# Twilight-Dream-Of-Magic/KolmogorovLike-DataCompressor

Hardware: AMD Instinct MI355X
Metric: compress MB/s at fixed block size, bit-exact vs reference; 1/2/4/8-GPU scaling (higher is better)
Workload: dtype u8; 1 GPU; enwik-style synthetic text (kolm.datagen.enwik_like, seed 20251212+rank), 256 MiB per GPU resident in HBM, 1 MiB fixed blocks, candidates 0..8 + MDL, payloads emitted in HBM; block_size=1048576, bytes_per_gpu=268435456, blocks_per_gpu=256, parallelism=block-shard x1

## Files before the change

### kolmogorovlike-datacompressor_amd/csrc/k_mtf.hip

```cpp
#include "kolm_internal.h"

namespace kolm {

namespace {

struct ChunkGeom {
    Geom geo;
    u32 cpb;
    u32 csz;
    __device__ inline bool range(u32 c, u32& lo, u32& hi) const {
        const u32 b = c / cpb;
        const u32 k = c - b * cpb;
        lo = geo.base(b) + k * csz;
        const u32 e = geo.end(b);
        hi = min(lo + csz, e);
        return lo < e;
    }
};

constexpr u32 MTF_SLAB = 64;

__global__ __launch_bounds__(256) void k_mtf_summary(ChunkGeom cg, const u8* in, u8* summary,
                                                     u16* scnt, u32 nchunks) {
    __shared__ u32 sl[256 * MTF_SLAB / 4];
    __shared__ u32 slo[256];
    const u32 t = threadIdx.x;
    const u32 c = blockIdx.x * blockDim.x + t;
    u32 lo = 0, hi = 0;
    const bool valid = c < nchunks && cg.range(c, lo, hi);
    u16 cnt = 0;
    if (__syncthreads_and(valid && hi - lo == cg.csz && (lo & 15) == 0)) {
        u32 seen[8] = {0, 0, 0, 0, 0, 0, 0, 0};
        u8* out = summary + (u64)c * 256;
        slo[t] = lo;
        __syncthreads();
        for (u32 r = cg.csz; r > 0; r -= MTF_SLAB) {
#pragma unroll
            for (u32 q = 0; q < MTF_SLAB / 16; ++q) {
                const u32 m = q * 256 + t, owner = m >> 2, part = m & 3;
                reinterpret_cast<uint4*>(sl)[m] =
                    *reinterpret_cast<const uint4*>(in + slo[owner] + r - MTF_SLAB + 16 * part);
            }
            __syncthreads();
            const u32* slab = sl + t * (MTF_SLAB / 4);
#pragma unroll
            for (int q = MTF_SLAB / 4 - 1; q >= 0; --q) {
                const u32 wv = slab[q];
#pragma unroll
                for (int j = 3; j >= 0; --j) {
                    const u32 b = (wv >> (8 * j)) & 0xFF, w = b >> 5, bit = 1u << (b & 31);
                    u32 sw = 0;
#pragma unroll
                    for (int k = 0; k < 8; ++k) sw = (k == (int)w) ? seen[k] : sw;
                    if (!(sw & bit)) {
#pragma unroll
                        for (int k = 0; k < 8; ++k)
                            if (k == (int)w) seen[k] |= bit;
                        out[cnt++] = (u8)b;
                    }
                }
            }
            __syncthreads();
        }
        scnt[c] = cnt;
        return;
    }
    if (!valid) {
        if (c < nchunks) scnt[c] = 0;
        return;
    }
    {
        u32 seen[8] = {0, 0, 0, 0, 0, 0, 0, 0};
        u8* out = summary + (u64)c * 256;
        auto visit = [&](u32 b) {
            const u32 w = b >> 5, bit = 1u << (b & 31);
            u32 sw = 0;
#pragma unroll
            for (int k = 0; k < 8; ++k) sw = (k == (int)w) ? seen[k] : sw;
            if (!(sw & bit)) {
#pragma unroll
                for (int k = 0; k < 8; ++k)
                    if (k == (int)w) seen[k] |= bit;
                out[cnt++] = (u8)b;
            }
        };
        if (((lo | hi) & 15) == 0) {
            for (u32 i = hi; i > lo; i -= 16) {
                const uint4 v = *reinterpret_cast<const uint4*>(in + i - 16);
                const u32 wv[4] = {v.x, v.y, v.z, v.w};
#pragma unroll
                for (int q = 3; q >= 0; --q)
#pragma unroll
                    for (int j = 3; j >= 0; --j) visit((wv[q] >> (8 * j)) & 0xFF);
            }
        } else {
            for (u32 i = hi; i > lo; --i) visit(in[i - 1]);
        }
    }
    scnt[c] = cnt;
}

__device__ inline void mtf_apply(u32* st, u8* nst, u32* member, const u8* sm, u32 cnt) {
    const u32 lane = threadIdx.x & 63;
    if (lane < 8) member[lane] = 0;
    __builtin_amdgcn_wave_barrier();
    __builtin_amdgcn_fence(__ATOMIC_RELEASE, "wavefront");
    u32 sv[4];
#pragma unroll
    for (int j = 0; j < 4; ++j) {
        const u32 i = 4 * lane + j;
        sv[j] = i < cnt ? sm[i] : 0;
        if (i < cnt) atomicOr(&member[sv[j] >> 5], 1u << (sv[j] & 31));
    }
    __builtin_amdgcn_fence(__ATOMIC_ACQ_REL, "wavefront");
    __builtin_amdgcn_wave_barrier();
    const u32 word = st[lane];
    u32 keep = 0;
    u8 e[4];
#pragma unroll
    for (int j = 0; j < 4; ++j) {
        e[j] = (word >> (8 * j)) & 0xFF;
        const bool in_sum = (member[e[j] >> 5] >> (e[j] & 31)) & 1u;
        keep |= (in_sum ? 0u : 1u) << j;
    }
    const u32 nk = __popc(keep);
    u32 pos = cnt + wave_incl_scan(nk, OpAddU(), 0u) - nk;
#pragma unroll
    for (int j = 0; j < 4; ++j) {
        const u32 i = 4 * lane + j;
        if (i < cnt) nst[i] = (u8)sv[j];
        if ((keep >> j) & 1u) nst[pos++] = e[j];
    }
    __builtin_amdgcn_fence(__ATOMIC_ACQ_REL, "wavefront");
    __builtin_amdgcn_wave_barrier();
    st[lane] = reinterpret_cast<const u32*>(nst)[lane];
    __builtin_amdgcn_fence(__ATOMIC_ACQ_REL, "wavefront");
    __builtin_amdgcn_wave_barrier();
}


constexpr u32 CP_W = 16;
constexpr u32 CP_G = 8;
constexpr u32 CP_S = 16;
constexpr u32 CP_R = CP_G * CP_S;

__device__ inline u32 mtf_ident(u32 lane) {
    return (4 * lane) | ((4 * lane + 1) << 8) | ((4 * lane + 2) << 16) | ((4 * lane + 3) << 24);
}

__device__ inline void cp_range(const ChunkGeom& cg, u32 b, u32 r, u32& k0, u32& k1) {
    const u32 nch = (cg.geo.end(b) - cg.geo.base(b) + cg.csz - 1) / cg.csz;
    const u32 per = (nch + CP_R - 1) / CP_R;
    k0 = min(r * per, nch);
    k1 = min(k0 + per, nch);
}

__global__ __launch_bounds__(64 * CP_W) void k_mtf_cp1(ChunkGeom cg, const u8* summary, const u16* scnt, u32* rst,
                                                      u32* rdist) {
    __shared__ u32 st[CP_W][64];
    __shared__ u8 nst[CP_W][256];
    __shared__ u32 member[CP_W][8];
    __shared__ u32 uni[CP_W][8];
    const u32 lane = threadIdx.x & 63, w = threadIdx.x >> 6;
    const u32 gr = blockIdx.x * CP_W + w, b = gr / CP_R, r = gr - b * CP_R;
    if (b >= cg.geo.nb) return;
    u32 k0, k1;
    cp_range(cg, b, r, k0, k1);
    st[w][lane] = mtf_ident(lane);
    if (lane < 8) uni[w][lane] = 0;
    __builtin_amdgcn_wave_barrier();
    for (u32 k = k0; k < k1; ++k) {
        const u32 c = b * cg.cpb + k;
        const u8* sm = summary + (u64)c * 256;
        const u32 cnt = scnt[c];
#pragma unroll
        for (int j = 0; j < 4; ++j) {
            const u32 i = 4 * lane + j;
            if (i < cnt) atomicOr(&uni[w][sm[i] >> 5], 1u << (sm[i] & 31));
        }
        mtf_apply(st[w], nst[w], member[w], sm, cnt);
    }
    __builtin_amdgcn_fence(__ATOMIC_ACQ_REL, "wavefront");
    __builtin_amdgcn_wave_barrier();
    rst[(u64)gr * 64 + lane] = st[w][lane];
    if (lane == 0) {
        u32 d = 0;
        for (int q = 0; q < 8; ++q) d += __popc(uni[w][q]);
        rdist[gr] = d;
    }
}

__global__ __launch_bounds__(64 * CP_G) void k_mtf_cp2(const u32* rst, const u32* rdist, u32* rentry) {
    __shared__ u32 st[CP_G][64];
    __shared__ u8 nst[CP_G][256];
    __shared__ u32 member[CP_G][8];
    __shared__ u32 uni[CP_G][8];
    __shared__ u8 gsum[CP_G][256];
    __shared__ u32 gentry[CP_G][64];
    __shared__ u32 gdist[CP_G];
    const u32 lane = threadIdx.x & 63, g = threadIdx.x >> 6, b = blockIdx.x;
    const u64 r0 = (u64)b * CP_R + g * CP_S;
    st[g][lane] = mtf_ident(lane);
    if (lane < 8) uni[g][lane] = 0;
    __builtin_amdgcn_wave_barrier();
    for (u32 v = 0; v < CP_S; ++v) {
        const u8* sm = reinterpret_cast<const u8*>(rst + (r0 + v) * 64);
        const u32 cnt = rdist[r0 + v];
#pragma unroll
        for (int j = 0; j < 4; ++j) {
            const u32 i = 4 * lane + j;
            if (i < cnt) atomicOr(&uni[g][sm[i] >> 5], 1u << (sm[i] & 31));
        }
        mtf_apply(st[g], nst[g], member[g], sm, cnt);
    }
    __builtin_amdgcn_fence(__ATOMIC_ACQ_REL, "wavefront");
    __builtin_amdgcn_wave_barrier();
    reinterpret_cast<u32*>(gsum[g])[lane] = st[g][lane];
    if (lane == 0) {
        u32 d = 0;
        for (int q = 0; q < 8; ++q) d += __popc(uni[g][q]);
        gdist[g] = d;
    }
    __syncthreads();
    if (g == 0) {
        st[0][lane] = mtf_ident(lane);
        __builtin_amdgcn_wave_barrier();
        for (u32 v = 0; v < CP_G; ++v) {
            gentry[v][lane] = st[0][lane];
            __builtin_amdgcn_fence(__ATOMIC_ACQ_REL, "wavefront");
            __builtin_amdgcn_wave_barrier();
            if (v + 1 < CP_G) mtf_apply(st[0], nst[0], member[0], gsum[v], gdist[v]);
        }
    }
    __syncthreads();
    st[g][lane] = gentry[g][lane];
    __builtin_amdgcn_wave_barrier();
    for (u32 v = 0; v < CP_S; ++v) {
        rentry[(r0 + v) * 64 + lane] = st[g][lane];
        mtf_apply(st[g], nst[g], member[g], reinterpret_cast<const u8*>(rst + (r0 + v) * 64), rdist[r0 + v]);
    }
}

__global__ __launch_bounds__(64 * CP_W) void k_mtf_cp3(ChunkGeom cg, const u8* summary, const u16* scnt,
                                                      const u32* rentry, u8* states) {
    __shared__ u32 st[CP_W][64];
    __shared__ u8 nst[CP_W][256];
    __shared__ u32 member[CP_W][8];
    const u32 lane = threadIdx.x & 63, w = threadIdx.x >> 6;
    const u32 gr = blockIdx.x * CP_W + w, b = gr / CP_R, r = gr - b * CP_R;
    if (b >= cg.geo.nb) return;
    u32 k0, k1;
    cp_range(cg, b, r, k0, k1);
    st[w][lane] = rentry[(u64)gr * 64 + lane];
    __builtin_amdgcn_wave_barrier();
    for (u32 k = k0; k < k1; ++k) {
        const u32 c = b * cg.cpb + k;
        reinterpret_cast<u32*>(states + (u64)c * 256)[lane] = st[w][lane];
        mtf_apply(st[w], nst[w], member[w], summary + (u64)c * 256, scnt[c]);
    }
}

constexpr int RT = 128;

struct RiceAcc {
    u32 c[5] = {0, 0, 0, 0, 0};
    int k;
    u32 kk = 0, km = 0;
    __device__ inline void init(int rk) {
        k = rk;
        kk = rk < 8 ? (u32)rk : 0u;
        km = rk < 8 ? (0xFFu >> rk) * 0x01010101u : 0u;
    }
    __device__ inline u32 rb(u32 v) const { return (v >> k) + 1 + k; }
    __device__ inline u32 sum4(u32 w, u32 a) const { return __builtin_amdgcn_sad_u8((w >> kk) & km, 0u, a); }
    __device__ inline void add(u32 v) {
        c[0] += rb(v);
        c[2] += rb(((v & 0x0Fu) << 4) | (v >> 4));
        c[3] += rb(__brev(v) >> 24);
        c[4] += rb(v ^ (v >> 1));
    }
    __device__ inline void add4(u32 o) {
        const u32 one = 4 * (1 + k);
        c[0] = sum4(o, c[0] + one);
        c[2] = sum4(((o & 0x0F0F0F0Fu) << 4) | ((o >> 4) & 0x0F0F0F0Fu), c[2] + one);
        c[3] = sum4(__brev(o), c[3] + one);
        c[4] = sum4(o ^ ((o >> 1) & 0x7F7F7F7Fu), c[4] + one);
    }
    __device__ inline void group(u32 lo, u32 hi) {
        u64 x = ((u64)__builtin_bswap32(lo) << 32) | __builtin_bswap32(hi);
        u64 t = (x ^ (x >> 7)) & 0x00AA00AA00AA00AAull;
        x ^= t ^ (t << 7);
        t = (x ^ (x >> 14)) & 0x0000CCCC0000CCCCull;
        x ^= t ^ (t << 14);
        t = (x ^ (x >> 28)) & 0x00000000F0F0F0F0ull;
        x ^= t ^ (t << 28);
        c[1] = sum4((u32)(x >> 32), sum4((u32)x, c[1] + 8 * (1 + k)));
    }
};

__global__ __launch_bounds__(RT) void k_mtf_replay(ChunkGeom cg, const u8* in, const u8* states, u8* out,
                                                   u32 nchunks, u64* bits, int rice_k) {
    __shared__ u32 tab[64 * RT];
    const u32 t = threadIdx.x;
    const u32 c = blockIdx.x * RT + t;
    u32 lo = 0, hi = 0;
    const bool valid = c < nchunks && cg.range(c, lo, hi);
    u32 r0 = 0, r1 = 0;
    if (valid) {
        const u32* s = reinterpret_cast<const u32*>(states + (u64)c * 256);
        r0 = s[0];
        r1 = s[1];
        for (int w = 2; w < 64; ++w) tab[w * RT + t] = s[w];
    }
    auto haszero = [](u32 y) { return (y - 0x01010101u) & ~y & 0x80808080u; };
    auto front = [](u32 x, u32 j, u32 in) {
        const u32 lowmask = j ? ((1u << (8 * j)) - 1) : 0u;
        const u32 highmask = j == 3 ? 0u : ~((1u << (8 * (j + 1))) - 1);
        return (x & highmask) | ((x & lowmask) << 8) | in;
    };
    auto step = [&](u32 b) -> u32 {
        const u32 bb = b * 0x01010101u;
        u32 z = haszero(r0 ^ bb);
        if (z) {
            const u32 j = (__ffs(z) - 1) >> 3;
            r0 = front(r0, j, b);
            return j;
        }
        const u32 c0 = r0 >> 24;
        z = haszero(r1 ^ bb);
        if (z) {
            const u32 j = (__ffs(z) - 1) >> 3;
            r0 = (r0 << 8) | b;
            r1 = front(r1, j, c0);
            return 4 + j;
        }
        u32 w = 2, x;
        for (;;) {
            x = tab[w * RT + t];
            z = haszero(x ^ bb);
            if (z) break;
            ++w;
        }
        const u32 j = (__ffs(z) - 1) >> 3;
        u32 carry = r1 >> 24;
        r1 = (r1 << 8) | c0;
        r0 = (r0 << 8) | b;
        for (u32 v = 2; v < w; ++v) {
            const u32 xv = tab[v * RT + t];
            tab[v * RT + t] = (xv << 8) | carry;
            carry = xv >> 24;
        }
        tab[w * RT + t] = front(x, j, carry);
        return 4 * w + j;
    };
    RiceAcc acc;
    acc.init(rice_k);
    if (!valid) return;
    if (((lo | hi) & 63) == 0) {
        for (u32 i = lo; i < hi; i += 64) {
            uint4 v[4];
#pragma unroll
            for (int h = 0; h < 4; ++h) v[h] = *reinterpret_cast<const uint4*>(in + i + 16 * h);
            u32 ov[16];
#pragma unroll
            for (int q = 0; q < 16; ++q) {
                const u32 wq = q % 4 == 0 ? v[q / 4].x : q % 4 == 1 ? v[q / 4].y : q % 4 == 2 ? v[q / 4].z : v[q / 4].w;
                u32 o = 0;
#pragma unroll
                for (int j = 0; j < 4; ++j) o |= step((wq >> (8 * j)) & 0xFF) << (8 * j);
                ov[q] = o;
                if (bits) acc.add4(o);
                if (bits && (q & 1)) acc.group(ov[q - 1], o);
            }
#pragma unroll
            for (int h = 0; h < 4; ++h)
                *reinterpret_cast<uint4*>(out + i + 16 * h) = make_uint4(ov[4 * h], ov[4 * h + 1], ov[4 * h + 2], ov[4 * h + 3]);
        }
    } else if (((lo | hi) & 15) == 0) {
        for (u32 i = lo; i < hi; i += 16) {
            const uint4 v = *reinterpret_cast<const uint4*>(in + i);
            const u32 wv[4] = {v.x, v.y, v.z, v.w};
            u32 ov[4];
#pragma unroll
            for (int q = 0; q < 4; ++q) {
                u32 o = 0;
#pragma unroll
                for (int j = 0; j < 4; ++j) o |= step((wv[q] >> (8 * j)) & 0xFF) << (8 * j);
                ov[q] = o;
                if (bits) acc.add4(o);
            }
            *reinterpret_cast<uint4*>(out + i) = make_uint4(ov[0], ov[1], ov[2], ov[3]);
            if (bits) {
                acc.group(ov[0], ov[1]);
                acc.group(ov[2], ov[3]);
            }
        }
    } else {
        u32 g[2] = {0, 0}, gi = 0;
        for (u32 i = lo; i < hi; ++i) {
            const u32 m = step(in[i]);
            out[i] = (u8)m;
            if (bits) {
                acc.add(m);
                g[gi >> 2] |= m << (8 * (gi & 3));
                if (++gi == 8) {
                    acc.group(g[0], g[1]);
                    g[0] = g[1] = 0;
                    gi = 0;
                }
            }
        }
        if (bits && gi) acc.group(g[0], g[1]);
    }
    if (bits) {
        u64* dst = bits + (u64)(c / cg.cpb) * 8;
#pragma unroll
        for (int q = 0; q < 5; ++q)
            if (acc.c[q]) atomicAdd((unsigned long long*)&dst[q], (unsigned long long)acc.c[q]);
    }
}

__global__ __launch_bounds__(256) void k_mtf_wave(ChunkGeom cg, const u8* in, const u8* states, u8* out,
                                                  u32 nchunks, u64* bits, int rice_k) {
    __shared__ u32 st[4][64];
    __shared__ u8 nst[4][256];
    __shared__ u32 member[4][8];
    __shared__ u8 inv[4][256];
    __shared__ u8 smy[4][64];
    __shared__ __align__(8) u8 mb[4][64];
    const u32 w = threadIdx.x >> 6, lane = threadIdx.x & 63;
    const u32 c = blockIdx.x * 4 + w;
    u32 lo = 0, hi = 0;
    if (!(c < nchunks && cg.range(c, lo, hi))) return;
    {
        const u32 word = reinterpret_cast<const u32*>(states + (u64)c * 256)[lane];
        st[w][lane] = word;
#pragma unroll
        for (int j = 0; j < 4; ++j) inv[w][(word >> (8 * j)) & 0xFF] = (u8)(4 * lane + j);
    }
    __builtin_amdgcn_fence(__ATOMIC_ACQ_REL, "wavefront");
    __builtin_amdgcn_wave_barrier();
    RiceAcc acc;
    acc.init(rice_k);
    const u64 below = (1ull << lane) - 1ull;
    for (u32 p = lo; p < hi; p += 64) {
        const u32 i = p + lane;
        const bool v = i < hi;
        const u32 sym = v ? in[i] : 0u;
        const u64 vm = __ballot(v);
        const u32 mypos = inv[w][sym];
        u64 rem = vm, mine = 0;
        while (rem) {
            const u32 k = (u32)__ffsll((long long)rem) - 1;
            const u32 sk = __builtin_amdgcn_readlane(sym, k);
            const u64 eq = __ballot(v && sym == sk);
            if (sym == sk) mine = eq;
            rem &= ~eq;
        }
        const u64 pm = mine & below;
        const u32 prev = pm ? 63u - (u32)__clzll((long long)pm) : 0u;
        const u64 win = pm ? below & ~((2ull << prev) - 1ull) : 0ull;
        u32 cnt = 0, seen = 0, less = 0;
        rem = vm;
        while (rem) {
            const u32 k = (u32)__ffsll((long long)rem) - 1;
            const u32 sk = __builtin_amdgcn_readlane(sym, k);
            const u32 pk = __builtin_amdgcn_readlane(mypos, k);
            const u64 eq = __ballot(v && sym == sk);
            cnt += (eq & win) ? 1u : 0u;
            if (k < lane) {
                ++seen;
                less += pk < mypos ? 1u : 0u;
            }
            rem &= ~eq;
        }
        const u32 m = pm ? cnt : seen + mypos - less;
        if (v) out[i] = (u8)m;
        mb[w][lane] = v ? (u8)m : (u8)0;
        if (bits && v) acc.add(m);
        const bool last = v && (mine >> lane) == 1ull;
        const u64 lm = __ballot(last);
        if (last) smy[w][__popcll(lm >> lane) - 1] = (u8)sym;
        __builtin_amdgcn_fence(__ATOMIC_ACQ_REL, "wavefront");
        __builtin_amdgcn_wave_barrier();
        if (bits && (lane & 7) == 0 && v) {
            const u32* g = reinterpret_cast<const u32*>(&mb[w][lane]);
            acc.group(g[0], g[1]);
        }
        mtf_apply(st[w], nst[w], member[w], smy[w], (u32)__popcll(lm));
        const u32 word = st[w][lane];
#pragma unroll
        for (int j = 0; j < 4; ++j) inv[w][(word >> (8 * j)) & 0xFF] = (u8)(4 * lane + j);
        __builtin_amdgcn_fence(__ATOMIC_ACQ_REL, "wavefront");
        __builtin_amdgcn_wave_barrier();
    }
    if (bits) {
        u64* dst = bits + (u64)(c / cg.cpb) * 8;
#pragma unroll
        for (int q = 0; q < 5; ++q) {
            const u32 sum = wave_reduce(acc.c[q], OpAddU(), 0u);
            if (lane == 0 && sum) atomicAdd((unsigned long long*)&dst[q], (unsigned long long)sum);
        }
    }
}

}

bool mtf_wave_mode(const Geom& geo) {
    const char* e = getenv("KOLM_MTF_WAVE");
    const int force = e ? atoi(e) : -1;
    return force >= 0 ? force != 0 : geo.nb < 64;
}

u32 mtf_chunk_bytes(const Geom& geo) {
    static const u32 force = getenv("KOLM_MTF_CHUNK") ? (u32)atoi(getenv("KOLM_MTF_CHUNK")) : 0u;
    if (force >= 64 && force <= MTF_CHUNK && (force & (force - 1)) == 0) return force;
    u32 csz = MTF_CHUNK;
    if (mtf_wave_mode(geo)) return csz;
    while (csz > 128 && (u64)((geo.bs + csz - 1) / csz) * geo.nb < 16384) csz >>= 1;
    return csz;
}

u64 mtf_cp_words(const Geom& geo) { return (u64)geo.nb * CP_R * 129; }

void launch_mtf(const Geom& geo, const u8* in, u8* out, u8* summary, u16* summary_cnt, u8* states,
                hipStream_t s, KTimer* kt, u64* bits, int rice_k, u32* cp_scratch) {
    if (!geo.N) return;
    const u32 csz = mtf_chunk_bytes(geo);
    ChunkGeom cg{geo, (geo.bs + csz - 1) / csz, csz};
    const u32 nchunks = cg.cpb * geo.nb;
    const u64 N = geo.N;
    {
        KScope k(kt, KT_MTF, "k_mtf_summary", N + (u64)nchunks * 256);
        k_mtf_summary<<<(nchunks + 255) / 256, 256, 0, s>>>(cg, in, summary, summary_cnt, nchunks);
    }
    {
        KScope k(kt, KT_MTF, "k_mtf_compose", (u64)nchunks * 512);
        {
            u32* rst = cp_scratch;
            u32* rentry = cp_scratch + (u64)geo.nb * CP_R * 64;
            u32* rdist = rentry + (u64)geo.nb * CP_R * 64;
            const u32 g13 = (geo.nb * CP_R + CP_W - 1) / CP_W;
            k_mtf_cp1<<<g13, 64 * CP_W, 0, s>>>(cg, summary, summary_cnt, rst, rdist);
            k_mtf_cp2<<<geo.nb, 64 * CP_G, 0, s>>>(rst, rdist, rentry);
            k_mtf_cp3<<<g13, 64 * CP_W, 0, s>>>(cg, summary, summary_cnt, rentry, states);
        }
    }
    if (mtf_wave_mode(geo)) {
        KScope k(kt, KT_MTF, "k_mtf_wave", 2 * N + (u64)nchunks * 256);
        k_mtf_wave<<<(nchunks + 3) / 4, 256, 0, s>>>(cg, in, states, out, nchunks, bits, rice_k);
    } else {
        KScope k(kt, KT_MTF, "k_mtf_replay", 2 * N + (u64)nchunks * 256);
        k_mtf_replay<<<(nchunks + RT - 1) / RT, RT, 0, s>>>(cg, in, states, out, nchunks, bits, rice_k);
    }
}

}
```

Before: 8634 MB/s.

## Rework MTF replay with 4-register head and branchless 16-byte window search

The per-thread MTF replay now keeps the first 16 list bytes in four registers and searches and shifts the rest in 4-word windows. Each window is updated with a branchless 128-bit mask instead of walking word by word through LDS. The chunk-prefix kernels now prefetch the next summary row into registers, track the distinct-symbol union inside mtf_apply instead of a separate atomic pass, and cp1/cp3 shrink from 16 to 4 waves per block. The wider windows cut loop iterations and LDS traffic on deep lookups, at the cost of extra ALU work and more register pressure.

```diff
diff --git a/kolmogorovlike-datacompressor_amd/csrc/k_mtf.hip b/kolmogorovlike-datacompressor_amd/csrc/k_mtf.hip
--- a/kolmogorovlike-datacompressor_amd/csrc/k_mtf.hip
+++ b/kolmogorovlike-datacompressor_amd/csrc/k_mtf.hip
@@ -1,4 +1,5 @@
 #include "kolm_internal.h"
+#include "mtf_core.h"
 
 namespace kolm {
 
@@ -100,7 +101,8 @@
     scnt[c] = cnt;
 }
 
-__device__ inline void mtf_apply(u32* st, u8* nst, u32* member, const u8* sm, u32 cnt) {
+template <bool UNI>
+__device__ inline void mtf_apply(u32* st, u8* nst, u32* member, u32 sw, u32 cnt, u32& seen) {
     const u32 lane = threadIdx.x & 63;
     if (lane < 8) member[lane] = 0;
     __builtin_amdgcn_wave_barrier();
@@ -109,11 +111,12 @@
 #pragma unroll
     for (int j = 0; j < 4; ++j) {
         const u32 i = 4 * lane + j;
-        sv[j] = i < cnt ? sm[i] : 0;
+        sv[j] = i < cnt ? (sw >> (8 * j)) & 0xFF : 0;
         if (i < cnt) atomicOr(&member[sv[j] >> 5], 1u << (sv[j] & 31));
     }
     __builtin_amdgcn_fence(__ATOMIC_ACQ_REL, "wavefront");
     __builtin_amdgcn_wave_barrier();
+    if (UNI && lane < 8) seen |= member[lane];
     const u32 word = st[lane];
     u32 keep = 0;
     u8 e[4];
@@ -138,8 +141,12 @@
     __builtin_amdgcn_wave_barrier();
 }
 
-
-constexpr u32 CP_W = 16;
+__device__ inline void mtf_apply(u32* st, u8* nst, u32* member, u32 sw, u32 cnt) {
+    u32 none = 0;
+    mtf_apply<false>(st, nst, member, sw, cnt, none);
+}
+
+constexpr u32 CP_W = 4;
 constexpr u32 CP_G = 8;
 constexpr u32 CP_S = 16;
 constexpr u32 CP_R = CP_G * CP_S;
@@ -155,72 +162,76 @@
     k1 = min(k0 + per, nch);
 }
 
+__device__ inline u32 mtf_set_size(u32 seen, u32 lane) {
+    return wave_reduce(lane < 8 ? (u32)__popc(seen) : 0u, OpAddU(), 0u);
+}
+
 __global__ __launch_bounds__(64 * CP_W) void k_mtf_cp1(ChunkGeom cg, const u8* summary, const u16* scnt, u32* rst,
                                                       u32* rdist) {
     __shared__ u32 st[CP_W][64];
     __shared__ u8 nst[CP_W][256];
     __shared__ u32 member[CP_W][8];
-    __shared__ u32 uni[CP_W][8];
     const u32 lane = threadIdx.x & 63, w = threadIdx.x >> 6;
     const u32 gr = blockIdx.x * CP_W + w, b = gr / CP_R, r = gr - b * CP_R;
     if (b >= cg.geo.nb) return;
     u32 k0, k1;
     cp_range(cg, b, r, k0, k1);
     st[w][lane] = mtf_ident(lane);
-    if (lane < 8) uni[w][lane] = 0;
-    __builtin_amdgcn_wave_barrier();
-    for (u32 k = k0; k < k1; ++k) {
-        const u32 c = b * cg.cpb + k;
-        const u8* sm = summary + (u64)c * 256;
-        const u32 cnt = scnt[c];
-#pragma unroll
-        for (int j = 0; j < 4; ++j) {
-            const u32 i = 4 * lane + j;
-            if (i < cnt) atomicOr(&uni[w][sm[i] >> 5], 1u << (sm[i] & 31));
-        }
-        mtf_apply(st[w], nst[w], member[w], sm, cnt);
+    __builtin_amdgcn_wave_barrier();
+    const u32* rows = reinterpret_cast<const u32*>(summary);
+    u64 c = (u64)b * cg.cpb + k0;
+    u32 cnt = 0, sw = 0, seen = 0;
+    if (k0 < k1) {
+        cnt = scnt[c];
+        sw = rows[c * 64 + lane];
+    }
+    for (u32 k = k0; k < k1; ++k, ++c) {
+        u32 ncnt = 0, nsw = 0;
+        if (k + 1 < k1) {
+            ncnt = scnt[c + 1];
+            nsw = rows[(c + 1) * 64 + lane];
+        }
+        mtf_apply<true>(st[w], nst[w], member[w], sw, cnt, seen);
+        cnt = ncnt;
+        sw = nsw;
     }
     __builtin_amdgcn_fence(__ATOMIC_ACQ_REL, "wavefront");
     __builtin_amdgcn_wave_barrier();
     rst[(u64)gr * 64 + lane] = st[w][lane];
-    if (lane == 0) {
-        u32 d = 0;
-        for (int q = 0; q < 8; ++q) d += __popc(uni[w][q]);
-        rdist[gr] = d;
-    }
+    const u32 d = mtf_set_size(seen, lane);
+    if (lane == 0) rdist[gr] = d;
 }
 
 __global__ __launch_bounds__(64 * CP_G) void k_mtf_cp2(const u32* rst, const u32* rdist, u32* rentry) {
     __shared__ u32 st[CP_G][64];
     __shared__ u8 nst[CP_G][256];
     __shared__ u32 member[CP_G][8];
-    __shared__ u32 uni[CP_G][8];
-    __shared__ u8 gsum[CP_G][256];
+    __shared__ u32 gsum[CP_G][64];
     __shared__ u32 gentry[CP_G][64];
     __shared__ u32 gdist[CP_G];
     const u32 lane = threadIdx.x & 63, g = threadIdx.x >> 6, b = blockIdx.x;
     const u64 r0 = (u64)b * CP_R + g * CP_S;
     st[g][lane] = mtf_ident(lane);
-    if (lane < 8) uni[g][lane] = 0;
-    __builtin_amdgcn_wave_barrier();
-    for (u32 v = 0; v < CP_S; ++v) {
-        const u8* sm = reinterpret_cast<const u8*>(rst + (r0 + v) * 64);
-        const u32 cnt = rdist[r0 + v];
-#pragma unroll
-        for (int j = 0; j < 4; ++j) {
-            const u32 i = 4 * lane + j;
-            if (i < cnt) atomicOr(&uni[g][sm[i] >> 5], 1u << (sm[i] & 31));
-        }
-        mtf_apply(st[g], nst[g], member[g], sm, cnt);
+    __builtin_amdgcn_wave_barrier();
+    u32 seen = 0;
+    {
+        u32 cnt = rdist[r0], sw = rst[r0 * 64 + lane];
+        for (u32 v = 0; v < CP_S; ++v) {
+            u32 ncnt = 0, nsw = 0;
+            if (v + 1 < CP_S) {
+                ncnt = rdist[r0 + v + 1];
+                nsw = rst[(r0 + v + 1) * 64 + lane];
+            }
+            mtf_apply<true>(st[g], nst[g], member[g], sw, cnt, seen);
+            cnt = ncnt;
+            sw = nsw;
+        }
     }
     __builtin_amdgcn_fence(__ATOMIC_ACQ_REL, "wavefront");
     __builtin_amdgcn_wave_barrier();
-    reinterpret_cast<u32*>(gsum[g])[lane] = st[g][lane];
-    if (lane == 0) {
-        u32 d = 0;
-        for (int q = 0; q < 8; ++q) d += __popc(uni[g][q]);
-        gdist[g] = d;
-    }
+    gsum[g][lane] = st[g][lane];
+    const u32 d = mtf_set_size(seen, lane);
+    if (lane == 0) gdist[g] = d;
     __syncthreads();
     if (g == 0) {
         st[0][lane] = mtf_ident(lane);
@@ -229,15 +240,25 @@
             gentry[v][lane] = st[0][lane];
             __builtin_amdgcn_fence(__ATOMIC_ACQ_REL, "wavefront");
             __builtin_amdgcn_wave_barrier();
-            if (v + 1 < CP_G) mtf_apply(st[0], nst[0], member[0], gsum[v], gdist[v]);
+            if (v + 1 < CP_G) mtf_apply(st[0], nst[0], member[0], gsum[v][lane], gdist[v]);
         }
     }
     __syncthreads();
     st[g][lane] = gentry[g][lane];
     __builtin_amdgcn_wave_barrier();
-    for (u32 v = 0; v < CP_S; ++v) {
-        rentry[(r0 + v) * 64 + lane] = st[g][lane];
-        mtf_apply(st[g], nst[g], member[g], reinterpret_cast<const u8*>(rst + (r0 + v) * 64), rdist[r0 + v]);
+    {
+        u32 cnt = rdist[r0], sw = rst[r0 * 64 + lane];
+        for (u32 v = 0; v < CP_S; ++v) {
+            u32 ncnt = 0, nsw = 0;
+            if (v + 1 < CP_S) {
+                ncnt = rdist[r0 + v + 1];
+                nsw = rst[(r0 + v + 1) * 64 + lane];
+            }
+            rentry[(r0 + v) * 64 + lane] = st[g][lane];
+            mtf_apply(st[g], nst[g], member[g], sw, cnt);
+            cnt = ncnt;
+            sw = nsw;
+        }
     }
 }
 
@@ -253,14 +274,33 @@
     cp_range(cg, b, r, k0, k1);
     st[w][lane] = rentry[(u64)gr * 64 + lane];
     __builtin_amdgcn_wave_barrier();
-    for (u32 k = k0; k < k1; ++k) {
-        const u32 c = b * cg.cpb + k;
-        reinterpret_cast<u32*>(states + (u64)c * 256)[lane] = st[w][lane];
-        mtf_apply(st[w], nst[w], member[w], summary + (u64)c * 256, scnt[c]);
+    const u32* rows = reinterpret_cast<const u32*>(summary);
+    u64 c = (u64)b * cg.cpb + k0;
+    u32 cnt = 0, sw = 0;
+    if (k0 < k1) {
+        cnt = scnt[c];
+        sw = rows[c * 64 + lane];
+    }
+    for (u32 k = k0; k < k1; ++k, ++c) {
+        u32 ncnt = 0, nsw = 0;
+        if (k + 1 < k1) {
+            ncnt = scnt[c + 1];
+            nsw = rows[(c + 1) * 64 + lane];
+        }
+        reinterpret_cast<u32*>(states + c * 256)[lane] = st[w][lane];
+        mtf_apply(st[w], nst[w], member[w], sw, cnt);
+        cnt = ncnt;
+        sw = nsw;
     }
 }
 
 constexpr int RT = 128;
+
+struct MtfColumn {
+    u32* col;
+    __device__ inline u32 load(u32 w) const { return col[(w - mtf::REG_WORDS) * RT]; }
+    __device__ inline void store(u32 w, u32 x) const { col[(w - mtf::REG_WORDS) * RT] = x; }
+};
 
 struct RiceAcc {
     u32 c[5] = {0, 0, 0, 0, 0};
@@ -300,58 +340,31 @@
 
 __global__ __launch_bounds__(RT) void k_mtf_replay(ChunkGeom cg, const u8* in, const u8* states, u8* out,
                                                    u32 nchunks, u64* bits, int rice_k) {
-    __shared__ u32 tab[64 * RT];
+    __shared__ u32 tab[(mtf::WORDS - mtf::REG_WORDS) * RT];
     const u32 t = threadIdx.x;
     const u32 c = blockIdx.x * RT + t;
     u32 lo = 0, hi = 0;
     const bool valid = c < nchunks && cg.range(c, lo, hi);
-    u32 r0 = 0, r1 = 0;
+    u32 r[4] = {0, 0, 0, 0};
+    const MtfColumn col{tab + t};
     if (valid) {
-        const u32* s = reinterpret_cast<const u32*>(states + (u64)c * 256);
-        r0 = s[0];
-        r1 = s[1];
-        for (int w = 2; w < 64; ++w) tab[w * RT + t] = s[w];
-    }
-    auto haszero = [](u32 y) { return (y - 0x01010101u) & ~y & 0x80808080u; };
-    auto front = [](u32 x, u32 j, u32 in) {
-        const u32 lowmask = j ? ((1u << (8 * j)) - 1) : 0u;
-        const u32 highmask = j == 3 ? 0u : ~((1u << (8 * (j + 1))) - 1);
-        return (x & highmask) | ((x & lowmask) << 8) | in;
-    };
-    auto step = [&](u32 b) -> u32 {
-        const u32 bb = b * 0x01010101u;
-        u32 z = haszero(r0 ^ bb);
-        if (z) {
-            const u32 j = (__ffs(z) - 1) >> 3;
-            r0 = front(r0, j, b);
-            return j;
-        }
-        const u32 c0 = r0 >> 24;
-        z = haszero(r1 ^ bb);
-        if (z) {
-            const u32 j = (__ffs(z) - 1) >> 3;
-            r0 = (r0 << 8) | b;
-            r1 = front(r1, j, c0);
-            return 4 + j;
-        }
-        u32 w = 2, x;
-        for (;;) {
-            x = tab[w * RT + t];
-            z = haszero(x ^ bb);
-            if (z) break;
-            ++w;
-        }
-        const u32 j = (__ffs(z) - 1) >> 3;
-        u32 carry = r1 >> 24;
-        r1 = (r1 << 8) | c0;
-        r0 = (r0 << 8) | b;
-        for (u32 v = 2; v < w; ++v) {
-            const u32 xv = tab[v * RT + t];
-            tab[v * RT + t] = (xv << 8) | carry;
-            carry = xv >> 24;
-        }
-        tab[w * RT + t] = front(x, j, carry);
-        return 4 * w + j;
+        const uint4* s = reinterpret_cast<const uint4*>(states + (u64)c * 256);
+        const uint4 h = s[0];
+        r[0] = h.x, r[1] = h.y, r[2] = h.z, r[3] = h.w;
+        for (u32 q = 1; q < 16; ++q) {
+            const uint4 v = s[q];
+            col.store(4 * q, v.x), col.store(4 * q + 1, v.y), col.store(4 * q + 2, v.z), col.store(4 * q + 3, v.w);
+        }
+    }
+    auto step = [&](u32 b) -> u32 { return mtf::step(r, col, b); };
+    auto step4 = [&](u32 wv) -> u32 {
+        u32 o = 0;
+#pragma nounroll
+        for (int j = 0; j < 4; ++j) {
+            o = (o >> 8) | (step(wv & 0xFF) << 24);
+            wv >>= 8;
+        }
+        return o;
     };
     RiceAcc acc;
     acc.init(rice_k);
@@ -365,9 +378,7 @@
 #pragma unroll
             for (int q = 0; q < 16; ++q) {
                 const u32 wq = q % 4 == 0 ? v[q / 4].x : q % 4 == 1 ? v[q / 4].y : q % 4 == 2 ? v[q / 4].z : v[q / 4].w;
-                u32 o = 0;
-#pragma unroll
-                for (int j = 0; j < 4; ++j) o |= step((wq >> (8 * j)) & 0xFF) << (8 * j);
+                const u32 o = step4(wq);
                 ov[q] = o;
                 if (bits) acc.add4(o);
                 if (bits && (q & 1)) acc.group(ov[q - 1], o);
@@ -383,9 +394,7 @@
             u32 ov[4];
 #pragma unroll
             for (int q = 0; q < 4; ++q) {
-                u32 o = 0;
-#pragma unroll
-                for (int j = 0; j < 4; ++j) o |= step((wv[q] >> (8 * j)) & 0xFF) << (8 * j);
+                const u32 o = step4(wv[q]);
                 ov[q] = o;
                 if (bits) acc.add4(o);
             }
@@ -426,7 +435,7 @@
     __shared__ u8 nst[4][256];
     __shared__ u32 member[4][8];
     __shared__ u8 inv[4][256];
-    __shared__ u8 smy[4][64];
+    __shared__ __align__(4) u8 smy[4][64];
     __shared__ __align__(8) u8 mb[4][64];
     const u32 w = threadIdx.x >> 6, lane = threadIdx.x & 63;
     const u32 c = blockIdx.x * 4 + w;
@@ -487,7 +496,8 @@
             const u32* g = reinterpret_cast<const u32*>(&mb[w][lane]);
             acc.group(g[0], g[1]);
         }
-        mtf_apply(st[w], nst[w], member[w], smy[w], (u32)__popcll(lm));
+        const u32 scnt = (u32)__popcll(lm);
+        mtf_apply(st[w], nst[w], member[w], 4 * lane < scnt ? reinterpret_cast<const u32*>(smy[w])[lane] : 0u, scnt);
         const u32 word = st[w][lane];
 #pragma unroll
         for (int j = 0; j < 4; ++j) inv[w][(word >> (8 * j)) & 0xFF] = (u8)(4 * lane + j);
diff --git a/kolmogorovlike-datacompressor_amd/csrc/mtf_core.h b/kolmogorovlike-datacompressor_amd/csrc/mtf_core.h
--- /dev/null
+++ b/kolmogorovlike-datacompressor_amd/csrc/mtf_core.h
@@ -0,0 +1,73 @@
+#pragma once
+#include <cstdint>
+
+#if defined(__HIPCC__)
+#define MTF_HD __host__ __device__ __forceinline__
+#else
+#define MTF_HD inline
+#endif
+
+namespace mtf {
+
+typedef uint32_t u32;
+typedef unsigned __int128 u128;
+
+constexpr u32 REG_WORDS = 4;
+constexpr u32 WORDS = 64;
+constexpr u32 TRIP = 4;
+
+MTF_HD u32 haszero(u32 y) { return (y - 0x01010101u) & ~y & 0x80808080u; }
+
+MTF_HD u32 popc(u32 x) {
+#if defined(__HIP_DEVICE_COMPILE__)
+    return (u32)__popc(x);
+#else
+    return (u32)__builtin_popcount(x);
+#endif
+}
+
+MTF_HD u32 front4(u32 x[4], u32 in, u32 bb, u32& carry) {
+    const u32 z0 = haszero(x[0] ^ bb), z1 = haszero(x[1] ^ bb), z2 = haszero(x[2] ^ bb), z3 = haszero(x[3] ^ bb);
+    const u128 Z = (u128)z0 | ((u128)z1 << 32) | ((u128)z2 << 64) | ((u128)z3 << 96);
+    const u128 below = Z ^ (Z - 1);
+    const u32 m[4] = {(u32)below, (u32)(below >> 32), (u32)(below >> 64), (u32)(below >> 96)};
+    const u32 s[4] = {(x[0] << 8) | in, (x[1] << 8) | (x[0] >> 24), (x[2] << 8) | (x[1] >> 24), (x[3] << 8) | (x[2] >> 24)};
+    carry = x[3] >> 24;
+#if defined(__HIP_DEVICE_COMPILE__)
+#pragma unroll
+#endif
+    for (int i = 0; i < 4; ++i) x[i] = (x[i] & ~m[i]) | (s[i] & m[i]);
+    const u32 n = (popc(m[0]) + popc(m[1]) + popc(m[2]) + popc(m[3])) >> 3;
+    return Z ? n : 0u;
+}
+
+template <class T>
+MTF_HD u32 trip(T& tab, u32 w, u32 bb, u32& carry) {
+    u32 x[TRIP], old[TRIP];
+#if defined(__HIP_DEVICE_COMPILE__)
+#pragma unroll
+#endif
+    for (u32 i = 0; i < TRIP; ++i) old[i] = x[i] = tab.load(w + i);
+    const u32 k = front4(x, carry, bb, carry);
+#if defined(__HIP_DEVICE_COMPILE__)
+#pragma unroll
+#endif
+    for (u32 i = 0; i < TRIP; ++i)
+        if (x[i] != old[i]) tab.store(w + i, x[i]);
+    return k;
+}
+
+template <class T>
+MTF_HD u32 step(u32 r[4], T& tab, u32 b) {
+    const u32 bb = b * 0x01010101u;
+    u32 carry;
+    const u32 n = front4(r, b, bb, carry);
+    if (n) return n - 1;
+    for (u32 w = REG_WORDS; w < WORDS; w += TRIP) {
+        const u32 k = trip(tab, w, bb, carry);
+        if (k) return 4 * w + k - 1;
+    }
+    return 255;
+}
+
+}
```

New measurement: 8598 MB/s. About the same (-0.4%).
